# pletzer/nemoflux

Hardware: AMD Instinct MI355X
Metric: edge-flux integrals/sec (higher is better)
Workload: dtype f64; 1 GPU; C4 ORCA12-like 3600x1800x75x12 in total (strong: 900 (t,z) slabs cut 1 way), psi=(1+10*z)*(t+1)*arctan2(y, x+180)/(2*pi), README singular transect + 64 node-snapped transects; nx=3600, ny=1800, nz=75, nt_global=12, target_segments=2229, weight_entries=15468144, parallelism=(t,z)-slab sharding x1, 1 all-reduce, resident_outputs=integratedVelocity [4][ncell] + |eU|,|eV| every step

## Files before the change

### nemoflux_amd/csrc/nf_capi_field.hip

```cpp
#include "nf_capi.h"

using namespace nf;

static int g_batch_steps = 1;
static long g_batch_cellsteps = 32l << 20;
static int g_partial_full = 0;
static int g_use_graph = 1;
static int g_inner_signed = 1;
static int g_k3_pairs = 1;
static int g_inner_interleaved = -1;
static int g_class_window = 32;
static int g_joint_window = 32;
static int g_joint_skip = 1;
static long g_knob_version = 0;

namespace nf {
int field_tuning_set(const char *name, int value)
{
    ++g_knob_version;
    if (!strcmp(name, "batch_steps")) {
        g_batch_steps = value;
        return NF_OK;
    }
    if (!strcmp(name, "batch_cellsteps_m")) {
        if (!(value >= 0 && value <= 2047)) return -1;
        g_batch_cellsteps = (long)value << 20;
        return NF_OK;
    }
    if (!strcmp(name, "partial_step_planes")) {
        g_partial_full = value != 0;
        return NF_OK;
    }
    if (!strcmp(name, "graph")) {
        g_use_graph = value != 0;
        return NF_OK;
    }
    if (!strcmp(name, "pass_inner_signed")) {
        g_inner_signed = value != 0;
        return NF_OK;
    }
    if (!strcmp(name, "pass_k3_pairs")) {
        g_k3_pairs = value != 0;
        return NF_OK;
    }
    if (!strcmp(name, "pass_inner_interleaved")) {
        if (!(value >= -1 && value <= 1)) return -1;
        g_inner_interleaved = value;
        return NF_OK;
    }
    if (!strcmp(name, "class_window")) {
        if (!(value >= 1 && value <= kClassWindowMax)) return -1;
        g_class_window = value;
        return NF_OK;
    }
    if (!strcmp(name, "joint_window")) {
        if (!(value >= 1 && value <= kClassWindowMax)) return -1;
        g_joint_window = value;
        return NF_OK;
    }
    if (!strcmp(name, "joint_skip")) {
        if (!(value == 0 || value == 1)) return -1;
        g_joint_skip = value;
        return NF_OK;
    }
    if (!strcmp(name, "area_chunk")) return area_chunk_set(value);
    if (!strcmp(name, "gross_chunk")) return gross_chunk_set(value);
    if (!strcmp(name, "crossing_chunk")) return crossing_chunk_set(value);
    return -1;
}
}

struct Series {
    const void *p[2] = {nullptr, nullptr};
    long nt = 0;
    int dtype = NF_F64, on_device = 1;
    double fill = std::numeric_limits<double>::quiet_NaN();
    double fill2 = std::numeric_limits<double>::quiet_NaN();
    DevArray<char> stage[2];
};

struct EdgeSet {
    std::vector<double> host;
    bool stale = false;
    DevArray<double> dev;
    int upload(size_t cap, hipStream_t s)
    {
        if (!stale) return NF_OK;
        NF_TRY(dev.reserve(cap));
        NF_HIP(hipMemcpyAsync(dev.get(), host.data(), sizeof(double) * host.size(), hipMemcpyHostToDevice, s));
        NF_HIP(hipStreamSynchronize(s));
        stale = false;
        return NF_OK;
    }
};

struct nf_field {
    hipStream_t stream = nullptr;
    long ny = 0, nx = 0, ncell = 0, nz = 0;
    struct Geometry {
        DevArray<double> xy, arc4, arcE, arcN;
        DevArray<unsigned long long> box;
        DevArray<double> iV;
        DevArray<double> abs;
        DevArray<double> aos;
        DevArray<double> pair[2];
        DevArray<double> tr_planes;
        DevArray<unsigned long long> maxbits;
        DevArray<double> iVb, absb, scratchb;
        DevArray<int> zr;
        long batch_steps = 0, batch_version = -1;
    } geo;
    double box[4] = {0, 0, 0, 0};
    DevArray<double> thick;
    Series uv;
    int sverdrup = 0;
    long s_begin = 0, s_end = -1;
    int compact = 0;
    bool derived_stale = false;
    std::vector<std::vector<double>> polylines;
    std::vector<int> poly_cc;
    std::vector<int> tr_off;
    WeightSet ws;
    bool weights_built = false;
    int skip_unsupported = 0;
    int overlap_warn = 0;
    DevArray<int> tr_off_dev;
    DevArray<double> scratch;
    DevArray<double> prof_scratch;
    DevArray<double> row;
    Series tau;
    double tau_ref = 0.0;
    int tau_wrap = 1;
    Series sig;
    Series e3;
    DevArray<char> e3u_static, e3v_static;
    long e3_static_nz = 0, e3_static_ny = 0, e3_static_nx = 0;
    DevArray<double> tprof_scratch;
    DevArray<double> area_scratch;
    DevArray<double> gross_scratch;
    DevArray<double> crossings;
    EdgeSet class_edges;
    DevArray<double> class_scratch;
    EdgeSet depth_edges;
    double depth_top = 0.0;
    struct Surfaces {
        const void *p[kMaxSurfaces] = {};
        int m = 0;
        long nt = 0;
        int dtype = NF_F64, on_device = 1;
        double fill = std::numeric_limits<double>::quiet_NaN();
        double fill2 = std::numeric_limits<double>::quiet_NaN();
        int wrap = 1;
        double top = 0.0;
        DevArray<char> fixed, stage;
        long fixed_ny = 0, fixed_nx = 0;
    } surf;
    EdgeSet joint_edges;
    int joint_na = 0, joint_nb = 0;
    DevArray<char> joint_table;
    DevArray<unsigned> joint_flags;
    DevArray<double> joint_scratch;
    Grid_t grid_view;
    bool timing = false;
    struct TimedLaunch {
        hipEvent_t e0 = nullptr, mid = nullptr, e1 = nullptr, e2 = nullptr;
        bool has_mid = false, has_k3 = false;
    };
    std::vector<TimedLaunch> ev;
    size_t ev_used = 0;
    long ev_dropped = 0;
    double last_flux_ms = 0.0, last_expand_ms = 0.0, last_k3_ms = 0.0;
    hipGraphExec_t graph_exec = nullptr;
    double *graph_rows = nullptr;
    long graph_version = -1, version = 0;
};

static long field_pass_version(const nf_field *f) { return f->version + tuning_version() + g_knob_version; }

static void field_drop_graph(nf_field *f)
{
    if (f->graph_exec) (void)hipGraphExecDestroy(f->graph_exec);
    f->graph_exec = nullptr;
    f->graph_rows = nullptr;
    f->graph_version = -1;
}

static int field_free_geometry(nf_field *f)
{
// ... 559 lines not shown
            snprintf(buf, sizeof buf, "%s: cannot allocate the term table of %zu bytes (%zu bytes x %zu records x %d owned levels)",
                     what, table_bytes, entry_bytes, nrec, lv.z1 - lv.z0);
            NF_REQUIRE(false, NF_ERR_HIP, buf);
        }
    }
    NF_TRY(f->joint_flags.reserve(blocks * (size_t)joint_flag_words((int)nrows, window)));
    NF_TRY(f->joint_scratch.reserve(nrec * (size_t)window));
    a->window = window;
    a->skip = g_joint_skip;
    a->table = f->joint_table.get();
    a->table_len = f->joint_table.size();
    a->flags = f->joint_flags.get();
    a->flags_len = f->joint_flags.size();
    a->scratch = f->joint_scratch.get();
    a->scratch_len = f->joint_scratch.size();
    return NF_OK;
}

static int field_joint_step_async(nf_field *f, long t, bool carry, double *rows_dev)
{
    const size_t nrows = field_joint_rows(f);
    Levels lv;
    NF_TRY(field_raw_step_begin(f, "compute_joint_class_transport", t, 2, rows_dev, nrows, &lv));
    if (lv.z1 <= lv.z0) return NF_OK;
    NF_TRY(f->joint_edges.upload(2 * (size_t)kMaxClassEdges, f->stream));
    JointArgs a;
    NF_TRY(field_joint_buffers(f, "compute_joint_class_transport", kJointEntryBytes, lv, nrows, &a));
    NF_TRY(field_step_input(f, t, lv, &a.in));
    NF_TRY(field_tracer_input(f, f->tau, t, lv, &a.ta));
    NF_TRY(field_tracer_input(f, f->sig, t, lv, &a.tb));
    a.carry = carry ? 1 : 0;
    a.edges = f->joint_edges.dev.get();
    a.na = f->joint_na;
    a.nb = f->joint_nb;
    a.tr = field_transects(f);
    a.rows = rows_dev;
    return launch_joint_class_transport(a, f->stream);
}

static int field_gross_class_async(nf_field *f, long t, bool carry, double *rows_dev)
{
    const int nedges = (int)f->class_edges.host.size();
    const size_t nrows = 2 * ((size_t)nedges + 2);
    Levels lv;
    NF_TRY(field_raw_step_begin(f, "compute_gross_class_transport", t, 2, rows_dev, nrows, &lv));
    if (lv.z1 <= lv.z0) return NF_OK;
    NF_TRY(f->class_edges.upload((size_t)kMaxClassEdges, f->stream));
    GrossClassArgs a;
    NF_TRY(field_joint_buffers(f, "compute_gross_class_transport", kJointEntryBytes, lv, nrows, &a));
    NF_TRY(field_step_input(f, t, lv, &a.in));
    NF_TRY(field_tracer_input(f, f->tau, t, lv, &a.cls));
    if (carry) a.carry = a.cls;
    if (f->sig.p[0]) NF_TRY(field_tracer_input(f, f->sig, t, lv, &a.cls));
    NF_TRY(field_cell_thick(f, t, lv, &a.th));
    a.edges = f->class_edges.dev.get();
    a.nedges = nedges;
    a.tr = field_transects(f);
    a.rows = rows_dev;
    return launch_gross_class_transport(a, f->stream);
}

static int field_class_area_async(nf_field *f, long t, double *rows_dev)
{
    const int nedges = (int)f->class_edges.host.size();
    const size_t nrows = 2 * ((size_t)nedges + 2);
    Levels lv;
    NF_TRY(field_raw_step_begin(f, "compute_class_area", t, 2, rows_dev, nrows, &lv));
    if (lv.z1 <= lv.z0) return NF_OK;
    NF_TRY(f->class_edges.upload((size_t)kMaxClassEdges, f->stream));
    ClassAreaArgs a;
    NF_TRY(field_joint_buffers(f, "compute_class_area", kClassAreaEntryBytes, lv, nrows, &a));
    NF_TRY(field_step_input(f, t, lv, &a.in));
    NF_TRY(field_tracer_input(f, f->tau, t, lv, &a.carry));
    a.cls = a.carry;
    if (f->sig.p[0]) NF_TRY(field_tracer_input(f, f->sig, t, lv, &a.cls));
    NF_TRY(field_cell_thick(f, t, lv, &a.th));
    a.edges = f->class_edges.dev.get();
    a.nedges = nedges;
    a.tr = field_transects(f);
    a.rows = rows_dev;
    return launch_class_area(a, f->stream);
}

static int field_pair_async(nf_field *f, long t, double *rows_dev, bool last, bool last_pair, bool interleaved)
{
    const int rowlen = field_row_length(f);
    StepForm first, second;
    first.inner = true;
    first.pair_buf = f->geo.pair[0].get();
    first.interleaved = interleaved;
    second.inner = g_inner_signed && !last;
    if (interleaved && second.inner && !last_pair) {
        second.pair_buf = f->geo.pair[1].get();
        second.interleaved = true;
    }
    NF_TRY(field_step_async(f, t, nullptr, first));
    NF_TRY(field_step_async(f, t + 1, nullptr, second));
    const double *uvB = second.pair_buf ? second.pair_buf : f->geo.iV.get() + f->ncell;
    NF_TRY(launch_integral_pair(field_transects(f), first.pair_buf, uvB, f->ncell, f->nx, f->scratch.get(),
                                rows_dev + (size_t)t * rowlen, rowlen, f->stream, first.interleaved, second.interleaved));
    NF_TRY(field_timed_k3_end(f));
    return NF_OK;
}

static long batch_cell_steps() { return g_batch_cellsteps; }

static bool field_can_batch(const nf_field *f)
{
    return g_batch_steps && !f->e3.p[0] && f->uv.on_device && f->uv.nt >= 2 && f->uv.nt < 65536 &&
           f->uv.nt * f->ncell <= batch_cell_steps() && f->ncell <= (1l << 20) && f->weights_built;
}

static bool field_pass_pairs(const nf_field *f)
{
    if (!g_k3_pairs || integral_uses_edges() || !f->geo.pair[0].get() || !f->weights_built) return false;
    const size_t step_bytes = (size_t)f->nz * f->ncell * elem_size(f->uv.dtype);
    FluxArgs a{};
    a.u = f->uv.on_device ? f->uv.p[0] : nullptr;
    a.v = f->uv.on_device ? f->uv.p[1] : nullptr;
    a.dtype = f->uv.dtype;
    a.ncell = f->ncell;
    return flux_supports_signed_only(a) && (!f->uv.on_device || step_bytes % 16 == 0);
}

static bool field_pass_interleaved(const nf_field *f)
{
    const bool on = g_inner_interleaved < 0 ? f->uv.dtype == NF_F64 : g_inner_interleaved != 0;
    if (!on || f->compact || f->e3.p[0]) return false;
    FluxArgs a{};
    a.u = f->uv.on_device ? f->uv.p[0] : nullptr;
    a.v = f->uv.on_device ? f->uv.p[1] : nullptr;
    a.dtype = f->uv.dtype;
    a.ncell = f->ncell;
    return flux_supports_interleaved(a);
}

static int field_prepare_pass(nf_field *f)
{
    if (!g_k3_pairs || integral_uses_edges() || !f->geo.iV.get()) return NF_OK;
    const PassSteps p = field_pass_steps(f);
    if (p.wb - p.wa < 2) return NF_OK;
    if (!f->geo.pair[0].get()) NF_TRY(f->geo.pair[0].alloc((size_t)f->ncell * 2));
    if (!f->geo.pair[1].get() && p.wb - p.wa >= 4 && field_pass_interleaved(f)) NF_TRY(f->geo.pair[1].alloc((size_t)f->ncell * 2));
    return NF_OK;
}

static int field_zero_unowned_rows(nf_field *f, double *rows_dev)
{
    const int rowlen = field_row_length(f);
    const PassSteps p = field_pass_steps(f);
    if (rowlen <= 0) return NF_OK;
    if (p.ta > 0) NF_HIP(hipMemsetAsync(rows_dev, 0, sizeof(double) * rowlen * (size_t)p.ta, f->stream));
    if (p.tb < f->uv.nt)
        NF_HIP(hipMemsetAsync(rows_dev + (size_t)p.tb * rowlen, 0, sizeof(double) * rowlen * (size_t)(f->uv.nt - p.tb),
                              f->stream));
    return NF_OK;
}

static int field_all_steps_direct(nf_field *f, double *rows_dev, bool zero_rows = true)
{
    const int rowlen = field_row_length(f);
    const PassSteps p = field_pass_steps(f);
    if (zero_rows) NF_TRY(field_zero_unowned_rows(f, rows_dev));
    const bool pairs = field_pass_pairs(f) && rowlen > 0;
    const long pa = pairs ? p.wa + (p.wb - p.wa) % 2 : p.wb;
    const bool interleaved = pairs && field_pass_interleaved(f) && (p.wb - pa < 4 || f->geo.pair[1].get());
    for (long t = p.ta; t < p.tb;) {
        const bool last = t + 1 == p.tb;
        if (t >= pa && t + 1 < p.wb) {
            NF_TRY(field_pair_async(f, t, rows_dev, t + 2 == p.tb, t + 2 == p.wb, interleaved));
            t += 2;
        } else {
            StepForm form;
            form.inner = g_inner_signed && !last;
            NF_TRY(field_step_async(f, t, rows_dev + (size_t)t * rowlen, form));
            t += 1;
        }
    }
    return NF_OK;
}

static int field_all_steps_batched(nf_field *f, double *rows_dev)
{
    const int rowlen = field_row_length(f);
    const size_t n = (size_t)f->ncell;
    nf_field::Geometry &g = f->geo;
    if (g.batch_steps != f->uv.nt) {
        NF_TRY(g.iVb.alloc(n * 4 * f->uv.nt));
        NF_TRY(g.absb.alloc(n * 2 * f->uv.nt));
        NF_TRY(g.zr.alloc((size_t)2 * f->uv.nt));
        NF_HIP(hipMemsetAsync(g.iVb.get(), 0, sizeof(double) * n * 4 * f->uv.nt, f->stream));
        g.batch_steps = f->uv.nt;
        g.batch_version = -1;
    }
    if (g.batch_version != f->version) {
        NF_TRY(g.scratchb.alloc((size_t)std::max(f->ws.nrec, f->ws.nent) * f->uv.nt));
        std::vector<int> zr((size_t)2 * f->uv.nt);
        for (long t = 0; t < f->uv.nt; ++t) {
            const Levels lv = field_levels(f, t);
            zr[2 * t] = lv.z0;
            zr[2 * t + 1] = lv.z1;
        }
        NF_HIP(hipMemcpy(g.zr.get(), zr.data(), sizeof(int) * zr.size(), hipMemcpyHostToDevice));
        g.batch_version = f->version;
    }
    StepInput in;
    NF_TRY(field_step_input(f, 0, {0, (int)f->nz}, &in));
    FluxArgs a = flux_args(in);
    a.iV = g.iVb.get();
    a.absU = g.absb.get();
    a.absV = g.absb.get() + f->ncell;
    a.maxbits = g.maxbits.get();
    a.batch.nsteps = (int)f->uv.nt;
    a.batch.in_stride = f->nz * f->ncell;
    a.batch.zr = g.zr.get();
    NF_TRY(field_launch_flux(f, a));
    if (rowlen > 0) {
        NF_TRY(field_integral(f, g.iVb.get(), g.scratchb.get(), rows_dev, (int)f->uv.nt, (long)(4 * n), rowlen));
        NF_TRY(field_timed_k3_end(f));
    }
    NF_HIP(hipMemcpyAsync(g.iV.get(), g.iVb.get() + (size_t)(f->uv.nt - 1) * 4 * n, sizeof(double) * 4 * n,
                          hipMemcpyDeviceToDevice, f->stream));
    NF_HIP(hipMemcpyAsync(g.abs.get(), g.absb.get() + (size_t)(f->uv.nt - 1) * 2 * n, sizeof(double) * 2 * n,
                          hipMemcpyDeviceToDevice, f->stream));
    f->derived_stale = false;
    return NF_OK;
}

extern "C" {

int nf_field_new(nf_field **self)
try {
    NF_REQUIRE(self, NF_ERR_ARG, "nf_field_new: null argument");
    *self = new nf_field();
    return NF_OK;
}
NF_API_CATCH
int nf_field_del(nf_field **self)
try {
    if (self && *self) {
        nf_field *f = *self;
        field_drop_events(f);
        field_drop_graph(f);
        delete f;
        *self = nullptr;
    }
    return NF_OK;
}
NF_API_CATCH
int nf_field_set_stream(nf_field **self, void *hip_stream)
try {
    NF_REQUIRE(self && *self, NF_ERR_ARG, "nf_field_set_stream: null field");
    (*self)->stream = (hipStream_t)hip_stream;
    ++(*self)->version;
// ... 1155 lines not shown
```

### nemoflux_amd/csrc/nf_common.h

```cpp
#pragma once
#include <hip/hip_runtime.h>
#include <cstdint>
#include <cstdio>
#include <string>
#include <cmath>
#include <initializer_list>
#include <mutex>
#include <vector>

#include "../../include/nemoflux_amd.h"

namespace nf {

constexpr int kWave = 64;
constexpr int kBlock = 256;
constexpr int kXcds = 8;
constexpr double kDeg2Rad = 3.14159265358979323846 / 180.0;
constexpr double kEarthRadiusSv = 6371000.0;

void set_error(const std::string &msg);
int hip_fail(hipError_t e, const char *what, const char *file, int line);

#define NF_HIP(call)                                                   \
    do {                                                               \
// ... 137 lines not shown
    }
    ~DevArray() { reset(); }
    int alloc(size_t n)
    {
        reset();
        void *q = nullptr;
        NF_HIP(hipMalloc(&q, n ? sizeof(T) * n : (sizeof(T) > 16 ? sizeof(T) : 16)));
        p_ = static_cast<T *>(q);
        n_ = n ? n : 1;
        return NF_OK;
    }
    int reserve(size_t n, bool *grown = nullptr)
    {
        const bool g = n_ == 0 || n_ < n;
        if (grown) *grown = g;
        return g ? alloc(n) : NF_OK;
    }
    void reset()
    {
        if (p_) (void)hipFree(p_);
        p_ = nullptr, n_ = 0;
    }
    T *get() const { return p_; }
    size_t size() const { return n_; }

private:
    T *p_ = nullptr;
    size_t n_ = 0;
};

struct WeightSet {
    long nrec = 0;
    DevArray<int> cell;
    DevArray<double> w4;
    DevArray<int> seg;
    DevArray<double> tab;
    int nseg = 0;
    DevArray<int> seg_start;
    std::vector<double> coverage;
    int over_seg = -1;
    long dropped = 0;
    struct EdgeEntry {
        int elem;
        int seg;
        double w;
    };
    long nent = 0;
    DevArray<EdgeEntry> ent;
    DevArray<int> ent_start;
    long entries() const { return 4 * nrec; }
    void release() { *this = WeightSet(); }
};
int fold_weights(WeightSet *ws, long ncell, long nx, hipStream_t s);
int weights_to_host(const WeightSet &ws, int64_t *cell_edge, double *weight, int *seg);
struct Box4;
struct LocatorBoxes {
    std::vector<DevArray<Box4>> level;
    std::vector<long> count;
    const double *xy = nullptr;
    long ncell = 0;
    double period = -1.0;
    std::mutex mtx;
    void release();
};
int build_weights(const double *xy, long ncell, const double *segs_host, const int *seg_cc_host, int nseg,
                  double periodX, WeightSet *out, hipStream_t s, int skip_unsupported = 0, int overlap_warn = 0,
                  LocatorBoxes *boxes = nullptr, long row_length = 0);
void weights_trim_scratch();

struct Transects {
    const WeightSet *ws = nullptr;
    const int *tr_offsets_dev = nullptr;
    int ntransect = 0;
    long row_length() const { return ws->nseg + ntransect; }
};

void integral_use_edges(int on);
int integral_uses_edges();
int launch_integral(const WeightSet &ws, const double *data, long ncell, int planes, long nx,
                    const int *tr_offsets_dev, int ntransect, double *scratch, double *row, hipStream_t s,
                    int nsteps = 1, long data_stride = 0, long row_stride = 0, const int *rec_cells = nullptr);
int launch_integral_pair(const Transects &tr, const double *uvA, const double *uvB, long ncell, long nx, double *scratch,
                         double *row, long row_stride, hipStream_t s, bool a_interleaved = false, bool b_interleaved = false);

struct StepInput {
    const void *u = nullptr, *v = nullptr;
    int dtype = NF_F64;
    long ncell = 0, ny = 0, nx = 0;
    int z0 = 0, z1 = 0;
    const double *thickness = nullptr, *arcE = nullptr, *arcN = nullptr;
    double fill = __builtin_nan(""), fill2 = __builtin_nan("");
    double scale = 1.0;
    int sverdrup = 0;
};

struct CellThick {
    const void *e3u = nullptr, *e3v = nullptr;
    double fill = __builtin_nan(""), fill2 = __builtin_nan("");
};
template <typename T>
struct ThickIn {
    const T *e3u, *e3v;
    T m1, m2;
};
template <typename T>
inline ThickIn<T> thick_in(const CellThick &c) { return ThickIn<T>{(const T *)c.e3u, (const T *)c.e3v, (T)c.fill, (T)c.fill2}; }
template <typename T>
__device__ inline double thick_fixed(T x, T m1, T m2)
{
    return (x != x || x == m1 || x == m2) ? 0.0 : (double)x;
}

struct TracerIn {
    const void *tau = nullptr;
    double fill = __builtin_nan(""), fill2 = __builtin_nan("");
    double ref = 0.0;
    int wrap_x = 1;
};

constexpr int kProfileChunk = 8;
constexpr int kCellThickProfileChunk = 4;
constexpr int kTracerProfileChunk = 4;
constexpr int kTracerProfileChunkF32 = 8;
inline int tracer_profile_chunk(int dtype) { return dtype == NF_F32 ? kTracerProfileChunkF32 : kTracerProfileChunk; }
struct ProfileArgs {
    StepInput in;
    Transects tr;
    double *scratch = nullptr;
    size_t scratch_len = 0;
    double *prof = nullptr;
    TracerIn t;
    CellThick th;
};
int launch_profile(const ProfileArgs &a, hipStream_t s);

constexpr int kAreaChunk = 4;
constexpr int kAreaChunkF32 = 8;
inline int area_chunk(int dtype) { return dtype == NF_F32 ? kAreaChunkF32 : kAreaChunk; }
int area_chunk_set(int levels);
int area_chunk_now(int dtype);
struct AreaArgs {
    StepInput in;
    Transects tr;
    double *scratch = nullptr;
    size_t scratch_len = 0;
    double *rows = nullptr;
    long nz = 0;
    TracerIn t;
    CellThick th;
};
int launch_area_profile(const AreaArgs &a, hipStream_t s);

constexpr int kGrossChunk = 8;
constexpr int kGrossChunkWideF64 = 4;
inline int gross_chunk(int dtype, bool carried, bool cell)
{
    return dtype == NF_F64 && (carried || cell) ? kGrossChunkWideF64 : kGrossChunk;
}
int gross_chunk_set(int levels);
int gross_chunk_now(int dtype, bool carried, bool cell);
struct GrossArgs {
    StepInput in;
    Transects tr;
    double *scratch = nullptr;
    size_t scratch_len = 0;
    double *rows = nullptr;
// ... 202 lines not shown
```

### nemoflux_amd/csrc/nf_integral.hip

```cpp
#include <type_traits>

#include "nf_common.h"

namespace nf {

typedef double dvec2 __attribute__((ext_vector_type(2)));

struct Record {
    long c;
    dvec2 wa, wb;
};
__device__ inline Record load_record(const int *__restrict__ cell, const double *__restrict__ w4, long k)
{
    const dvec2 *pw = reinterpret_cast<const dvec2 *>(w4 + 4 * k);
    return Record{__builtin_nontemporal_load(cell + k), __builtin_nontemporal_load(pw), __builtin_nontemporal_load(pw + 1)};
}
__device__ inline int load_key(const int *__restrict__ seg, long k) { return __builtin_nontemporal_load(seg + k); }

struct Neighbours {
    unsigned j, i;
    bool south;
    long cs, cw;
};
__device__ inline Neighbours neighbours(long c, unsigned nx)
// ... 253 lines not shown
        const int nlev = z1 - z < DL ? z1 - z : DL;
        LevelUV<T> x[DL];
        LevelTau<T> tt[TR ? DL : 1];
        LevelUV<T> e3[CT ? DL : 1];
#pragma unroll
        for (int l = 0; l < DL; ++l)
            if (l < nlev) {
                const long o = (long)(z + l) * ncell;
                x[l] = load_level_uv(u, v, o, r.c, nb);
                if constexpr (CT) e3[l] = load_level_e3(ct, o, r.c, nb);
                if constexpr (TR) tt[l] = load_level_tau(ti.tau, o, r.c, nb);
            }
#pragma unroll
        for (int l = 0; l < DL; ++l)
            if (l < nlev) {
                FaceTf tf{};
                if constexpr (TR) tf = level_tf(tt[l], nb, ti);
                SlotTh th;
                if constexpr (CT)
                    th = level_th(e3[l], ct);
                else
                    th = slot_th(thickness[z + l]);
                const Slots d = level_slots_tf<T, TR>(th, x[l], arc, fill, fill2, two, scale, sverdrup, nb.south, tf);
                const SlotTh Dn = below(D, th);
                level(D, Dn, d, nb.south);
                D = Dn;
            }
    }
}

__global__ __launch_bounds__(kBlock) void k_gather_segscan(const int *__restrict__ cell,
                                                           const double *__restrict__ w4,
                                                           const int *__restrict__ seg, long n,
                                                           const double *__restrict__ data, long ncell,
                                                           int planes, unsigned nx, double *__restrict__ runsum,
                                                           long data_stride)
{
    data += (long)blockIdx.y * data_stride;
    runsum += (long)blockIdx.y * n;
    const long k = (long)blockIdx.x * kBlock + threadIdx.x;
    double val[1] = {0.0};
    int key = -1;
    if (k < n) {
        const Record r = load_record(cell, w4, k);
        Slots d;
        if (planes == 2) {
            d = signed_plane_slots(data + ncell, ncell, r.c, neighbours(r.c, nx));
        } else if (planes) {
            d.s = data[r.c], d.e = data[ncell + r.c], d.n = data[2 * ncell + r.c], d.w = data[3 * ncell + r.c];
        } else {
            const double2 *pd = reinterpret_cast<const double2 *>(data + 4 * r.c);
            const double2 da = pd[0], db = pd[1];
            d = Slots{da.y, db.x, da.x, db.y};
        }
        val[0] = weighted_sum(r, d);
        key = load_key(seg, k);
    }
    if (seg_scan(val, key, k, n)) runsum[k] = val[0];
}

template <bool A_IL, bool B_IL>
__global__ __launch_bounds__(kBlock) void k_gather_segscan_pair(const int *__restrict__ cell, const double *__restrict__ w4,
                                                                const int *__restrict__ seg, long n,
                                                                const double *__restrict__ uvA,
                                                                const double *__restrict__ uvB, long ncell, unsigned nx,
                                                                double *__restrict__ runsum)
{
    const long k = (long)blockIdx.x * kBlock + threadIdx.x;
    double val[2] = {0.0, 0.0};
    int key = -1;
    if (k < n) {
        const Record r = load_record(cell, w4, k);
        const Neighbours nb = neighbours(r.c, nx);
        val[0] = weighted_sum(r, A_IL ? interleaved_slots(uvA, r.c, nb) : signed_plane_slots(uvA, ncell, r.c, nb));
        val[1] = weighted_sum(r, B_IL ? interleaved_slots(uvB, r.c, nb) : signed_plane_slots(uvB, ncell, r.c, nb));
        key = load_key(seg, k);
    }
    if (seg_scan(val, key, k, n)) {
        runsum[k] = val[0];
        runsum[n + k] = val[1];
    }
}

__global__ __launch_bounds__(kBlock) void k_gather_edges(const WeightSet::EdgeEntry *__restrict__ ent, long n,
                                                         const double *__restrict__ data, long ncell,
                                                         double *__restrict__ runsum, long data_stride)
{
    data += (long)blockIdx.y * data_stride + ncell;
    runsum += (long)blockIdx.y * n;
    const long k = (long)blockIdx.x * kBlock + threadIdx.x;
    double val[1] = {0.0};
    int key = -1;
    if (k < n) {
        typedef int ivec4 __attribute__((ext_vector_type(4)));
        const ivec4 r = __builtin_nontemporal_load(reinterpret_cast<const ivec4 *>(ent + k));
        double w;
        const int wbits[2] = {r.z, r.w};
        __builtin_memcpy(&w, wbits, 8);
        val[0] = w * data[(unsigned)r.x];
        key = r.y;
    }
    if (seg_scan(val, key, k, n)) runsum[k] = val[0];
}

__global__ __launch_bounds__(kBlock) void k_finalize_seg(const double *__restrict__ runsum,
                                                         const int *__restrict__ seg_start, int nseg,
                                                         double *__restrict__ row, long nrec, long row_stride)
{
    runsum += (long)blockIdx.y * nrec;
    row += (long)blockIdx.y * row_stride;
    const int s = (blockIdx.x * kBlock + threadIdx.x) / kWave;
    const int lane = threadIdx.x & (kWave - 1);
    if (s >= nseg) return;
    const long lo = seg_start[s], hi = seg_start[s + 1];
    double acc = 0.0;
    if (hi > lo) {
        const long w0 = lo / kWave, w1 = (hi - 1) / kWave;
        for (long w = w0 + lane; w <= w1; w += kWave) {
            long e = (w + 1) * kWave;
            if (e > hi) e = hi;
            acc += runsum[e - 1];
        }
    }
    for (int o = 32; o > 0; o >>= 1) acc += __shfl_xor(acc, o, kWave);
    if (lane == 0) row[s] = acc;
}

__global__ __launch_bounds__(kBlock) void k_finalize_tr(const int *__restrict__ tr_off, int ntransect, int nseg,
                                                        double *__restrict__ row, long row_stride)
{
    row += (long)blockIdx.y * row_stride;
    const int p = (blockIdx.x * kBlock + threadIdx.x) / kWave;
    const int lane = threadIdx.x & (kWave - 1);
    if (p >= ntransect) return;
    double part = 0.0;
    for (int s = tr_off[p] + lane; s < tr_off[p + 1]; s += kWave) part += row[s];
    for (int o = 32; o > 0; o >>= 1) part += __shfl_xor(part, o, kWave);
    if (lane == 0) row[nseg + p] = part;
}

static void launch_finalize(const Transects &tr, const int *run_start, long nrun, const double *runsum, double *row,
                            long row_stride, unsigned nrows, hipStream_t s)
{
    const int nseg = tr.ws->nseg;
    if (nseg > 0) {
        const unsigned nb = (unsigned)(((long)nseg * kWave + kBlock - 1) / kBlock);
        hipLaunchKernelGGL(k_finalize_seg, dim3(nb, nrows), dim3(kBlock), 0, s, runsum, run_start, nseg, row, nrun, row_stride);
    }
    if (tr.ntransect > 0) {
        const unsigned nb = (unsigned)(((long)tr.ntransect * kWave + kBlock - 1) / kBlock);
        hipLaunchKernelGGL(k_finalize_tr, dim3(nb, nrows), dim3(kBlock), 0, s, tr.tr_offsets_dev, tr.ntransect, nseg, row,
                           row_stride);
    }
}

static dim3 record_grid(const WeightSet &ws, unsigned ny = 1) { return dim3((unsigned)((ws.nrec + kBlock - 1) / kBlock), ny); }

static int g_use_edges = 0;
void integral_use_edges(int on) { g_use_edges = on; }
int integral_uses_edges() { return g_use_edges; }

int launch_integral(const WeightSet &ws, const double *data, long ncell, int planes, long nx,
                    const int *tr_offsets_dev, int ntransect, double *scratch, double *row, hipStream_t s, int nsteps,
                    long data_stride, long row_stride, const int *rec_cells)
{
    const Transects tr{&ws, tr_offsets_dev, ntransect};
    const unsigned ny = (unsigned)(nsteps > 1 ? nsteps : 1);
    const bool edges = planes == 2 && ws.ent_start.get() && g_use_edges;
    if (edges && ws.nent > 0)
        hipLaunchKernelGGL(k_gather_edges, dim3((unsigned)((ws.nent + kBlock - 1) / kBlock), ny), dim3(kBlock), 0, s,
                           ws.ent.get(), ws.nent, data, ncell, scratch, data_stride);
    if (!edges && ws.nrec > 0)
        hipLaunchKernelGGL(k_gather_segscan, record_grid(ws, ny), dim3(kBlock), 0, s,
                           rec_cells ? rec_cells : ws.cell.get(), ws.w4.get(), ws.seg.get(), ws.nrec, data, ncell, planes,
                           (unsigned)(nx > 0 ? nx : 1), scratch, data_stride);
    launch_finalize(tr, edges ? ws.ent_start.get() : ws.seg_start.get(), edges ? ws.nent : ws.nrec, scratch, row, row_stride,
                    ny, s);
    NF_HIP(hipGetLastError());
    return NF_OK;
}

int launch_integral_pair(const Transects &tr, const double *uvA, const double *uvB, long ncell, long nx, double *scratch,
                         double *row, long row_stride, hipStream_t s, bool a_interleaved, bool b_interleaved)
{
    const WeightSet &ws = *tr.ws;
    NF_REQUIRE(a_interleaved || !b_interleaved, NF_ERR_ARG, "integral: operand B is interleaved only when A is");
    if (ws.nrec > 0) {
        auto *kernel = b_interleaved ? k_gather_segscan_pair<true, true>
                                     : (a_interleaved ? k_gather_segscan_pair<true, false> : k_gather_segscan_pair<false, false>);
        hipLaunchKernelGGL(kernel, record_grid(ws), dim3(kBlock), 0, s, ws.cell.get(), ws.w4.get(), ws.seg.get(), ws.nrec,
                           uvA, uvB, ncell, (unsigned)(nx > 0 ? nx : 1), scratch);
    }
    launch_finalize(tr, ws.seg_start.get(), ws.nrec, scratch, row, row_stride, 2, s);
    NF_HIP(hipGetLastError());
    return NF_OK;
}

static int check_raw_step(const char *what, const StepInput &in, const Transects &tr, size_t scratch_len, size_t per_record)
{
    const std::string w(what);
    NF_REQUIRE(tr.ws && in.ncell > 0 && in.nx > 0 && in.ncell % in.nx == 0 && in.ncell < (1l << 31), NF_ERR_ARG,
               w + ": bad grid sizes");
    NF_REQUIRE(in.z0 >= 0 && in.z1 >= in.z0 && tr.ntransect >= 0, NF_ERR_ARG, w + ": bad arguments");
    NF_REQUIRE(scratch_len >= (size_t)tr.ws->nrec * per_record, NF_ERR_ARG, w + ": scratch too small");
    return NF_OK;
}

template <typename T, int LZ, typename... TI>
__global__ __launch_bounds__(kBlock) void k_profile_segscan(const int *__restrict__ cell, const double *__restrict__ w4,
                                                            const int *__restrict__ seg, long n, const T *__restrict__ u,
                                                            const T *__restrict__ v, long ncell, unsigned nx, int z0,
                                                            int nlev, const double *__restrict__ thickness,
                                                            const double *__restrict__ arcE,
                                                            const double *__restrict__ arcN, T fill, T fill2, int two,
                                                            double scale, int sverdrup, double *__restrict__ runsum,
                                                            TI... tracer)
{
    constexpr bool TR = (std::is_same<TI, TauIn<T>>::value || ...);
    constexpr bool CT = (std::is_same<TI, ThickIn<T>>::value || ...);
    const TauIn<T> ti = tau_in<T>(tracer...);
    const ThickIn<T> ct = thick_arg<T>(tracer...);
    const long k = (long)blockIdx.x * kBlock + threadIdx.x;
    double val[LZ];
#pragma unroll
    for (int l = 0; l < LZ; ++l) val[l] = 0.0;
    int key = -1;
    if (k < n) {
        const Record r = load_record(cell, w4, k);
        key = load_key(seg, k);
        const auto nb = step_neighbours<TR>(r.c, nx, ncell, ti.wrap_x);
        const Arcs arc = load_arcs(arcE, arcN, r.c, nb);
        LevelUV<T> x[LZ];
        LevelTau<T> tt[TR ? LZ : 1];
        LevelUV<T> e3[CT ? LZ : 1];
#pragma unroll
        for (int l = 0; l < LZ; ++l)
            if (l < nlev) {
                x[l] = load_level_uv(u, v, (long)(z0 + l) * ncell, r.c, nb);
                if constexpr (CT) e3[l] = load_level_e3(ct, (long)(z0 + l) * ncell, r.c, nb);
                if constexpr (TR) tt[l] = load_level_tau(ti.tau, (long)(z0 + l) * ncell, r.c, nb);
            }
#pragma unroll
        for (int l = 0; l < LZ; ++l)
            if (l < nlev) {
                FaceTf tf{};
                if constexpr (TR) tf = level_tf(tt[l], nb, ti);
                SlotTh th;
                if constexpr (CT)
                    th = level_th(e3[l], ct);
                else
                    th = slot_th(thickness[z0 + l]);
                val[l] = weighted_sum(r, level_slots_tf<T, TR>(th, x[l], arc, fill, fill2, two, scale, sverdrup, nb.south, tf));
            }
    }
    if (seg_scan(val, key, k, n)) {
#pragma unroll
        for (int l = 0; l < LZ; ++l)
            if (l < nlev) runsum[(long)l * n + k] = val[l];
    }
}


template <typename T, int FORM>
static int launch_profile_t(const ProfileArgs &a, hipStream_t s)
{
    constexpr bool TR = FORM == 1;
    constexpr int chunk = FORM == 2 ? kCellThickProfileChunk
                                    : !TR ? kProfileChunk : sizeof(T) == 4 ? kTracerProfileChunkF32 : kTracerProfileChunk;
    const WeightSet &ws = *a.tr.ws;
    const StepInput &in = a.in;
    const long row_length = a.tr.row_length();
    const T fill = (T)in.fill, fill2 = (T)in.fill2;
    for (int zc = in.z0; zc < in.z1; zc += chunk) {
        const int nlev = in.z1 - zc < chunk ? in.z1 - zc : chunk;
        if (ws.nrec > 0) {
            if constexpr (TR)
// ... 1392 lines not shown
```

Baseline: 385.5 billion integrals/s.

## Batch k3 transect integrals over groups of up to twelve time steps

Generalises the paired-step integral pass into groups of up to 12 consecutive steps. Each step's signed velocity plane goes to its own buffer, and one gather/segmented-scan kernel then loads each weight record, its neighbours and its scan masks once for all steps in the group. The aim is to cut repeated record and key loads and per-step kernel launches. In exchange it allocates more per-step plane buffers and a larger scratch area, with a fallback to pairs when allocation fails.

After: 387.4 billion integrals/s, median of 6. No clear change (+0.5%).

```diff
diff --git a/nemoflux_amd/csrc/nf_capi_field.hip b/nemoflux_amd/csrc/nf_capi_field.hip
--- a/nemoflux_amd/csrc/nf_capi_field.hip
+++ b/nemoflux_amd/csrc/nf_capi_field.hip
@@ -8,6 +8,7 @@
 static int g_use_graph = 1;
 static int g_inner_signed = 1;
 static int g_k3_pairs = 1;
+static int g_k3_group = 12;
 static int g_inner_interleaved = -1;
 static int g_class_window = 32;
 static int g_joint_window = 32;
@@ -41,6 +42,11 @@
     }
     if (!strcmp(name, "pass_k3_pairs")) {
         g_k3_pairs = value != 0;
+        return NF_OK;
+    }
+    if (!strcmp(name, "pass_k3_group")) {
+        if (!(value >= 1 && value <= kGroupMax)) return -1;
+        g_k3_group = value;
         return NF_OK;
     }
     if (!strcmp(name, "pass_inner_interleaved")) {
@@ -103,7 +109,8 @@
         DevArray<double> iV;
         DevArray<double> abs;
         DevArray<double> aos;
-        DevArray<double> pair[2];
+        std::vector<DevArray<double>> group;
+        int group_size = 1;
         DevArray<double> tr_planes;
         DevArray<unsigned long long> maxbits;
         DevArray<double> iVb, absb, scratchb;
@@ -829,23 +836,28 @@
     return launch_class_area(a, f->stream);
 }
 
-static int field_pair_async(nf_field *f, long t, double *rows_dev, bool last, bool last_pair, bool interleaved)
+static int field_group_async(nf_field *f, long t, int m, double *rows_dev, bool last, bool last_group, bool interleaved)
 {
     const int rowlen = field_row_length(f);
-    StepForm first, second;
-    first.inner = true;
-    first.pair_buf = f->geo.pair[0].get();
-    first.interleaved = interleaved;
-    second.inner = g_inner_signed && !last;
-    if (interleaved && second.inner && !last_pair) {
-        second.pair_buf = f->geo.pair[1].get();
-        second.interleaved = true;
-    }
-    NF_TRY(field_step_async(f, t, nullptr, first));
-    NF_TRY(field_step_async(f, t + 1, nullptr, second));
-    const double *uvB = second.pair_buf ? second.pair_buf : f->geo.iV.get() + f->ncell;
-    NF_TRY(launch_integral_pair(field_transects(f), first.pair_buf, uvB, f->ncell, f->nx, f->scratch.get(),
-                                rows_dev + (size_t)t * rowlen, rowlen, f->stream, first.interleaved, second.interleaved));
+    GroupSteps g;
+    g.nsteps = m;
+    for (int q = 0; q < m; ++q) {
+        StepForm form;
+        form.inner = q + 1 < m || (g_inner_signed && !last);
+        if (q + 1 < m || (interleaved && form.inner && !last_group)) {
+            form.pair_buf = f->geo.group[q].get();
+            form.interleaved = interleaved;
+        }
+        NF_TRY(field_step_async(f, t + q, nullptr, form));
+        g.uv[q] = form.pair_buf ? form.pair_buf : f->geo.iV.get() + f->ncell;
+        if (form.interleaved) g.interleaved |= 1u << q;
+    }
+    double *rows = rows_dev + (size_t)t * rowlen;
+    if (m == 2)
+        NF_TRY(launch_integral_pair(field_transects(f), g.uv[0], g.uv[1], f->ncell, f->nx, f->scratch.get(), rows, rowlen,
+                                    f->stream, g.interleaved & 1u, (g.interleaved >> 1) & 1u));
+    else
+        NF_TRY(launch_integral_group(field_transects(f), g, f->ncell, f->nx, f->scratch.get(), rows, rowlen, f->stream));
     NF_TRY(field_timed_k3_end(f));
     return NF_OK;
 }
@@ -858,9 +870,9 @@
            f->uv.nt * f->ncell <= batch_cell_steps() && f->ncell <= (1l << 20) && f->weights_built;
 }
 
-static bool field_pass_pairs(const nf_field *f)
-{
-    if (!g_k3_pairs || integral_uses_edges() || !f->geo.pair[0].get() || !f->weights_built) return false;
+static bool field_pass_can_group(const nf_field *f)
+{
+    if (!g_k3_pairs || g_k3_group < 2 || integral_uses_edges() || !f->weights_built || !f->geo.iV.get()) return false;
     const size_t step_bytes = (size_t)f->nz * f->ncell * elem_size(f->uv.dtype);
     FluxArgs a{};
     a.u = f->uv.on_device ? f->uv.p[0] : nullptr;
@@ -882,13 +894,39 @@
     return flux_supports_interleaved(a);
 }
 
+static size_t pass_group_buffers(long nw, int gs, bool interleaved)
+{
+    if (gs < 2 || nw < 2) return 0;
+    const long largest = std::min<long>(gs, nw), groups = nw / gs + (nw % gs >= 2 ? 1 : 0);
+    return (size_t)(interleaved && groups >= 2 ? largest : largest - 1);
+}
+
 static int field_prepare_pass(nf_field *f)
 {
-    if (!g_k3_pairs || integral_uses_edges() || !f->geo.iV.get()) return NF_OK;
+    nf_field::Geometry &g = f->geo;
+    g.group_size = 1;
     const PassSteps p = field_pass_steps(f);
-    if (p.wb - p.wa < 2) return NF_OK;
-    if (!f->geo.pair[0].get()) NF_TRY(f->geo.pair[0].alloc((size_t)f->ncell * 2));
-    if (!f->geo.pair[1].get() && p.wb - p.wa >= 4 && field_pass_interleaved(f)) NF_TRY(f->geo.pair[1].alloc((size_t)f->ncell * 2));
+    const long nw = p.wb - p.wa;
+    const bool il = field_pass_interleaved(f);
+    for (int gs : {std::min(g_k3_group, kGroupMax), 2}) {
+        if (!field_pass_can_group(f) || pass_group_buffers(nw, gs, il) == 0) break;
+        const size_t need = pass_group_buffers(nw, gs, il);
+        if (g.group.size() > need) g.group.resize(need);
+        bool ok = f->scratch.reserve((size_t)std::min<long>(gs, nw) * std::max(f->ws.nrec, f->ws.nent)) == NF_OK;
+        while (ok && g.group.size() < need) {
+            DevArray<double> buf;
+            ok = buf.alloc((size_t)f->ncell * 2) == NF_OK;
+            if (ok) g.group.push_back(std::move(buf));
+        }
+        if (ok) {
+            g.group_size = gs;
+            return NF_OK;
+        }
+        (void)hipGetLastError();
+        if (gs == 2) break;
+    }
+    g.group.clear();
+    if (f->weights_built && !f->scratch.get()) NF_TRY(f->scratch.alloc((size_t)2 * std::max(f->ws.nrec, f->ws.nent)));
     return NF_OK;
 }
 
@@ -909,14 +947,17 @@
     const int rowlen = field_row_length(f);
     const PassSteps p = field_pass_steps(f);
     if (zero_rows) NF_TRY(field_zero_unowned_rows(f, rows_dev));
-    const bool pairs = field_pass_pairs(f) && rowlen > 0;
-    const long pa = pairs ? p.wa + (p.wb - p.wa) % 2 : p.wb;
-    const bool interleaved = pairs && field_pass_interleaved(f) && (p.wb - pa < 4 || f->geo.pair[1].get());
+    const long nw = p.wb - p.wa;
+    const bool il = field_pass_interleaved(f);
+    int gs = rowlen > 0 && field_pass_can_group(f) ? f->geo.group_size : 1;
+    if (f->geo.group.size() < pass_group_buffers(nw, gs, il)) gs = 1;
+    const bool interleaved = gs >= 2 && il;
     for (long t = p.ta; t < p.tb;) {
         const bool last = t + 1 == p.tb;
-        if (t >= pa && t + 1 < p.wb) {
-            NF_TRY(field_pair_async(f, t, rows_dev, t + 2 == p.tb, t + 2 == p.wb, interleaved));
-            t += 2;
+        const int m = t >= p.wa && t < p.wb && gs >= 2 ? (int)((p.wb - t) % gs ? (p.wb - t) % gs : gs) : 1;
+        if (m >= 2) {
+            NF_TRY(field_group_async(f, t, m, rows_dev, t + m == p.tb, t + m == p.wb, interleaved));
+            t += m;
         } else {
             StepForm form;
             form.inner = g_inner_signed && !last;
diff --git a/nemoflux_amd/csrc/nf_common.h b/nemoflux_amd/csrc/nf_common.h
--- a/nemoflux_amd/csrc/nf_common.h
+++ b/nemoflux_amd/csrc/nf_common.h
@@ -243,6 +243,14 @@
                     int nsteps = 1, long data_stride = 0, long row_stride = 0, const int *rec_cells = nullptr);
 int launch_integral_pair(const Transects &tr, const double *uvA, const double *uvB, long ncell, long nx, double *scratch,
                          double *row, long row_stride, hipStream_t s, bool a_interleaved = false, bool b_interleaved = false);
+constexpr int kGroupMax = 16;
+struct GroupSteps {
+    const double *uv[kGroupMax] = {};
+    unsigned interleaved = 0;
+    int nsteps = 0;
+};
+int launch_integral_group(const Transects &tr, const GroupSteps &g, long ncell, long nx, double *scratch, double *row,
+                          long row_stride, hipStream_t s);
 
 struct StepInput {
     const void *u = nullptr, *v = nullptr;
diff --git a/nemoflux_amd/csrc/nf_integral.hip b/nemoflux_amd/csrc/nf_integral.hip
--- a/nemoflux_amd/csrc/nf_integral.hip
+++ b/nemoflux_amd/csrc/nf_integral.hip
@@ -359,6 +359,39 @@
     }
 }
 
+template <bool IN_IL, bool LAST_IL>
+__global__ __launch_bounds__(kBlock) void k_gather_segscan_group(const int *__restrict__ cell, const double *__restrict__ w4,
+                                                                 const int *__restrict__ seg, long n, const GroupSteps g,
+                                                                 long ncell, unsigned nx, double *__restrict__ runsum)
+{
+    const long k = (long)blockIdx.x * kBlock + threadIdx.x;
+    const int lane = threadIdx.x & (kWave - 1);
+    const bool has = k < n;
+    Record r{};
+    Neighbours nb{};
+    int key = -1;
+    if (has) {
+        r = load_record(cell, w4, k);
+        nb = neighbours(r.c, nx);
+        key = load_key(seg, k);
+    }
+    unsigned take = 0;
+#pragma unroll
+    for (int o = 1, b = 0; o < kWave; o <<= 1, ++b)
+        if (seg_scan_take(key, lane, o)) take |= 1u << b;
+    const bool store = seg_run_end(key, lane, k, n);
+    auto step = [&](int q, auto il) {
+        const double *uv = g.uv[q];
+        double val[1] = {0.0};
+        if (has) val[0] = weighted_sum(r, decltype(il)::value ? interleaved_slots(uv, r.c, nb) : signed_plane_slots(uv, ncell, r.c, nb));
+#pragma unroll
+        for (int o = 1, b = 0; o < kWave; o <<= 1, ++b) seg_scan_step(val, o, take & (1u << b));
+        if (store) runsum[(long)q * n + k] = val[0];
+    };
+    for (int q = 0; q + 1 < g.nsteps; ++q) step(q, std::integral_constant<bool, IN_IL>{});
+    step(g.nsteps - 1, std::integral_constant<bool, LAST_IL>{});
+}
+
 __global__ __launch_bounds__(kBlock) void k_gather_edges(const WeightSet::EdgeEntry *__restrict__ ent, long n,
                                                          const double *__restrict__ data, long ncell,
                                                          double *__restrict__ runsum, long data_stride)
@@ -469,6 +502,27 @@
                            uvA, uvB, ncell, (unsigned)(nx > 0 ? nx : 1), scratch);
     }
     launch_finalize(tr, ws.seg_start.get(), ws.nrec, scratch, row, row_stride, 2, s);
+    NF_HIP(hipGetLastError());
+    return NF_OK;
+}
+
+int launch_integral_group(const Transects &tr, const GroupSteps &g, long ncell, long nx, double *scratch, double *row,
+                          long row_stride, hipStream_t s)
+{
+    const WeightSet &ws = *tr.ws;
+    NF_REQUIRE(g.nsteps >= 1 && g.nsteps <= kGroupMax, NF_ERR_ARG, "integral: a group has 1 .. 16 steps");
+    for (int q = 0; q < g.nsteps; ++q) NF_REQUIRE(g.uv[q], NF_ERR_ARG, "integral: a step of the group has no buffer");
+    const unsigned inner = (1u << (g.nsteps - 1)) - 1, in_bits = g.interleaved & inner;
+    const bool in_il = g.nsteps > 1 ? in_bits == inner : (g.interleaved & 1u) != 0, last_il = (g.interleaved >> (g.nsteps - 1)) & 1u;
+    NF_REQUIRE(g.nsteps == 1 || in_bits == 0 || in_bits == inner, NF_ERR_ARG, "integral: the steps before the last share one form");
+    NF_REQUIRE(in_il || !last_il, NF_ERR_ARG, "integral: the last step is interleaved only when the others are");
+    if (ws.nrec > 0) {
+        auto *kernel = last_il ? k_gather_segscan_group<true, true>
+                               : (in_il ? k_gather_segscan_group<true, false> : k_gather_segscan_group<false, false>);
+        hipLaunchKernelGGL(kernel, record_grid(ws), dim3(kBlock), 0, s, ws.cell.get(), ws.w4.get(), ws.seg.get(), ws.nrec, g,
+                           ncell, (unsigned)(nx > 0 ? nx : 1), scratch);
+    }
+    launch_finalize(tr, ws.seg_start.get(), ws.nrec, scratch, row, row_stride, (unsigned)g.nsteps, s);
     NF_HIP(hipGetLastError());
     return NF_OK;
 }
```
